# Syclus123/xDeepFM-pytorch

Measured on AMD Instinct MI355X. Metric: examples/sec (xDeepFM train step, Criteo-shape synthetic, bs=4096 per GPU), higher is better.
Workload: dtype f32

## Files before the change

include/xdfm.h:

```cpp
#ifndef XDFM_H
#define XDFM_H

#include <stddef.h>
#include <stdint.h>

#ifdef __cplusplus
extern "C" {
#endif

#define XDFM_ABI_VERSION 8

enum {
    XDFM_OK = 0,
    XDFM_ERR_INVALID = 1,
    XDFM_ERR_LAUNCH = 2,
    XDFM_ERR_NO_DEVICE = 3
};

enum { XDFM_ACT_LINEAR = 0, XDFM_ACT_RELU = 1, XDFM_ACT_SIGMOID = 2 };

int xdfm_abi_version(void);
const char* xdfm_last_error(void);
int xdfm_device_count(void);
int xdfm_set_option(const char* key, int value);
// ... 62 lines not shown
int xdfm_cin_fwd_pack(const float* W, int H, int Hp, int m, float* Wf, void* stream);
int xdfm_cin_level_fwd(const float* xp, const float* x0, const float* Wf, const float* bias,
                       int H, int Hp, int m, long N, int act, float* out, void* stream);

int xdfm_cin_level_fwd_ex_supported(int H, int Hp, int m, int D);
int xdfm_cin_level_fwd_ex(const float* xp, const float* x0, const float* Wf, const float* bias, int H, int Hp, int m, long N,
                          int act, float* out, int keep_rows, float* res, long ldres, int res_off, int dir0, int D,
                          unsigned* mask, long mask_ld, void* stream);

int xdfm_cin_direct_sum(const float* A, int row0, int rows, int B, int D,
                        float* res, long ldres, int off, void* stream);

int xdfm_cin_dout(const float* A, int H, int B, int D, int act,
                  const float* dHid, int hid0, int hid_rows,
                  const float* dDir, int dir_mode, long lddir, int dir_off, int dir0, int dir_rows,
                  float* dOut, float* dbias, void* stream);
size_t xdfm_cin_dout_ws_elems(int H, int B, int D);
int xdfm_cin_dout_det(const float* A, int H, int B, int D, int act,
                  const float* dHid, int hid0, int hid_rows,
                  const float* dDir, int dir_mode, long lddir, int dir_off, int dir0, int dir_rows,
                  float* dOut, float* dbias, float* ws, void* stream);

size_t xdfm_cin_bwd_pack_elems(int H, int Hp, int m);
int xdfm_cin_bwd_pack(const float* W, int H, int Hp, int m, float* Wz, void* stream);
int xdfm_cin_level_bwd_x(const float* dOut, const float* xp, const float* x0, const float* Wz,
                         int H, int Hp, int m, long N, float* dxp, float* dx0, void* stream);
enum { XDFM_BWX_SET_DXP = 1, XDFM_BWX_SET_DX0 = 2 };
int xdfm_cin_level_bwd_x_ex(const float* dOut, const float* xp, const float* x0, const float* Wz, int H, int Hp,
                            int m, long N, float* dxp, float* dx0, int flags, void* stream);

int xdfm_cin_bwd_x_is_folded(int H, int Hp, int m, int xp_is_x0);

size_t xdfm_cin_bwd_w_ws_elems(int H, int Hp, int m, long N);
int xdfm_cin_level_bwd_w(const float* dOut, const float* xp, const float* x0,
                         int H, int Hp, int m, long N, float* ws, float* dW, void* stream);

size_t xdfm_cin_bwd_prep_ws_elems(int H, int Hp, int m, int B, int D);
int xdfm_cin_bwd_nodout_supported(int H, int Hp, int m, int B, int D);
int xdfm_cin_level_bwd_x_src(const unsigned* mask, long mask_ld, const float* dHid, int hid_rows, const float* dDir, int dir_mode,
                             long lddir, int dir_off, int dir0, int dir_rows, int D, int h0, const float* xp, const float* x0,
                             const float* Wz, int H, int Hp, int m, long N, float* dxp, float* dx0, int flags, void* stream);
int xdfm_cin_bwd_prep(const float* A, const unsigned* mask, long mask_ld, int H, int B, int D, int act, const float* dHid,
                      int hid0, int hid_rows, const float* dDir, int dir_mode, long lddir, int dir_off, int dir0, int dir_rows,
                      float* dOut, float* dbias, float* dout_ws, const float* xp, const float* x0, int Hp, int m, float* bww_ws,
                      int* prepared, void* stream);
int xdfm_cin_level_bwd_w_prepared(const float* dOut, const float* xp, const float* x0, int H, int Hp, int m, long N,
                                  float* ws, float* dW, void* stream);

size_t xdfm_cin_attn_theta_elems(int D, int n_layers, int use_ln);
int xdfm_cin_attn_pool_fwd(const float* fm, int B, int S, int D, int nh, int n_layers, int use_ln, int use_res,
                           const float* theta, float* out, float* tok_save, float* o_save, float* ml_save,
                           float p_drop, const unsigned long long* drop_seed, void* stream);
int xdfm_cin_attn_pool_bwd(const float* fm, int B, int S, int D, int nh, int n_layers, int use_ln, int use_res,
                           const float* theta, const float* tok_save, const float* o_save, const float* ml_save,
                           const float* dout, float* dfm, float* dtheta, float p_drop,
                           const unsigned long long* drop_seed, void* stream);
size_t xdfm_cin_attn_pool_bwd_ws_elems(int B, int D, int n_layers, int use_ln);
int xdfm_cin_attn_pool_bwd_det(const float* fm, int B, int S, int D, int nh, int n_layers, int use_ln, int use_res,
                               const float* theta, const float* tok_save, const float* o_save, const float* ml_save,
                               const float* dout, float* dfm, float* dtheta, float* ws, float p_drop,
                               const unsigned long long* drop_seed, void* stream);
int xdfm_cin_attn_dropout_mask(int B, int S, int nh, int n_layers, float p_drop, const unsigned long long* drop_seed,
                               unsigned char* keep, void* stream);

int xdfm_l2_reg_fwd(const float* const* ptrs, const long* numel, const float* coeff, int T,
                    float* partials, float* out, void* stream);
int xdfm_l2_reg_bwd(const float* const* ptrs, const long* numel, const float* coeff, int T,
                    const float* gscale, float* gflat, const long* goff, int accumulate, void* stream);

typedef struct {
    const float* W;
    int H, Hp, m;
    float* fwd_pack;
    float* bwd_pack;
} xdfm_cin_pack_job;
int xdfm_cin_pack_all_supported(int H, int Hp, int m);
int xdfm_cin_pack_all(const xdfm_cin_pack_job* jobs, int L, void* stream);

size_t xdfm_colsum_ws_elems(int cols);
int xdfm_colsum(const float* g, long rows, int cols, long ld, float* ws, float* out, void* stream);
int xdfm_relu_bwd_colsum(const float* g, const float* y, long rows, int cols, long ldg, long ldy, float* ws, float* gz,
                         float* out, void* stream);

enum { XDFM_LINK_SIGMOID = 0, XDFM_LINK_IDENTITY = 1 };
enum { XDFM_LOSS_BCE = 0, XDFM_LOSS_MSE = 1, XDFM_LOSS_MAE = 2 };
size_t xdfm_head_ws_elems(int Ku, int Kv);
int xdfm_head_fwd(const float* lin, const float* u, const float* wu, int Ku, const float* v, const float* wv, int Kv,
                  const float* bias, const float* y, int B, float* pred, float* loss, float* ws, void* stream);
int xdfm_head_bwd(const float* pred, const float* y, const float* gloss, const float* u, const float* wu, int Ku,
                  const float* v, const float* wv, int Kv, int B, float* dlin, float* du, float* dv, float* grads,
                  float* ws, void* stream);
int xdfm_head_fwd_ex(const float* lin, const float* u, const float* wu, int Ku, const float* v, const float* wv, int Kv,
                     const float* bias, const float* y, int B, float* pred, float* loss_out, float* ws, int link, int loss,
                     void* stream);
int xdfm_head_bwd_ex(const float* pred, const float* y, const float* gloss, const float* u, const float* wu, int Ku,
                     const float* v, const float* wv, int Kv, int B, float* dlin, float* du, float* dv, float* grads,
                     float* ws, int link, int loss, void* stream);

typedef struct {
    float* param;
    float* grad;
    float* exp_avg;
    float* exp_avg_sq;
    const float* step;
    long numel;
    float l2;
    unsigned char* grad_marks;
    int flags;
    unsigned char* last;
} xdfm_adam_tensor;
enum { XDFM_ADAM_LAZY = 1, XDFM_ADAM_DEFERRED = 2 };
size_t xdfm_adam_step_ws_elems(int T);
int xdfm_adam_step(const xdfm_adam_tensor* tensors, int T, double lr, double beta1, double beta2, double eps,
                   float* l2_ws, float* l2_value, void* stream);
int xdfm_adam_step_lr(const xdfm_adam_tensor* tensors, int T, double lr, const double* lr_dev, double beta1, double beta2,
                      double eps, float* l2_ws, float* l2_value, void* stream);

typedef struct {
    float* param;
    float* grad;
    float* state;
    long numel;
    float l2;
    unsigned char* grad_marks;
} xdfm_opt_tensor;
size_t xdfm_opt_step_ws_elems(int T);
int xdfm_sgd_step(const xdfm_opt_tensor* tensors, int T, double lr, const double* lr_dev, float* l2_ws, float* l2_value,
                  void* stream);
int xdfm_adagrad_step(const xdfm_opt_tensor* tensors, int T, double lr, const double* lr_dev, double eps, float* l2_ws,
                      float* l2_value, void* stream);
int xdfm_rmsprop_step(const xdfm_opt_tensor* tensors, int T, double lr, const double* lr_dev, double alpha, double eps,
                      float* l2_ws, float* l2_value, void* stream);

typedef struct {
    int* clock;
    float* consts;
    int cap;
} xdfm_adam_clock;
int xdfm_adam_step_deferred(const xdfm_adam_tensor* tensors, int T, const xdfm_adam_clock* clk, double lr,
                            const double* lr_dev, double beta1, double beta2, double eps, float* l2_ws, float* l2_value,
                            void* stream);
typedef struct {
    float* const* param;
    float* const* exp_avg;
    float* const* exp_avg_sq;
    unsigned char* const* last;
    const float* l2;
    float* const* grad;
    unsigned char* const* marks;
} xdfm_adam_rows;
int xdfm_adam_catchup_rows(const float* X, long ldx, int B, const int* cols, const int* vocab, int m, int D,
                           const xdfm_adam_rows* emb, const xdfm_adam_rows* lin, const xdfm_adam_clock* clk,
                           double beta1, double beta2, double eps, float* backlog, void* stream);
int xdfm_adam_apply_rows(const float* X, long ldx, int B, const int* cols, const int* vocab, int m, int D,
                         const xdfm_adam_rows* emb, const xdfm_adam_rows* lin, const xdfm_adam_clock* clk,
                         double beta1, double beta2, double eps, float* l2_cell, float* l2_value, void* stream);
int xdfm_adam_flush(const xdfm_adam_tensor* tensors, int T, const xdfm_adam_clock* clk, double beta1, double beta2,
                    double eps, float* backlog, void* stream);

typedef struct {
    int* clock;
    float* rates;
    int cap;
    unsigned long long* backlog;
    unsigned long long* cell;
} xdfm_opt_clock;
// ... 79 lines not shown
```

xdeepfm-pytorch_amd/xdfm_amd/_lib.py:

```python
import ctypes
import os
from ctypes import c_char_p, c_double, c_float, c_int, c_long, c_size_t, c_void_p

import torch

_HERE = os.path.dirname(os.path.abspath(__file__))
LIB_PATH = os.environ.get("XDFM_LIB", os.path.join(_HERE, "libxdfm_hip.so"))

P = c_void_p
SIGNATURES = {
    "xdfm_abi_version": (c_int, []),
    "xdfm_last_error": (c_char_p, []),
    "xdfm_device_count": (c_int, []),
    "xdfm_set_option": (c_int, [c_char_p, c_int]),
    "xdfm_get_option": (c_int, [c_char_p]),
    "xdfm_graph_node_census": (c_int, [P, P, P, P]),
    "xdfm_set_ticket_board": (c_int, [P, c_int]),
    "xdfm_embed_gather_fwd": (c_int, [P, c_long, c_int, P, P, P, P, c_int, c_int, P, P, c_int, P, P, P, P, P]),
    "xdfm_embed_gather_fwd_ld": (c_int, [P, c_long, c_int, P, P, P, P, c_int, c_int, P, P, c_int, P, P, c_long, c_int, P, P, P]),
    "xdfm_varlen_pool_fwd": (c_int, [P, c_long, c_int, P, P, c_int, c_int, c_int, P, P, c_long, c_int, P, P, P, P]),
    "xdfm_varlen_pool_bwd_ws_elems": (c_size_t, [c_long, c_int, c_int, c_int]),
    "xdfm_varlen_pool_bwd": (c_int, [P, c_long, c_int, P, P, c_int, c_int, c_int, P, P, c_long, c_int, P, c_long, P, P, P, P, P, P,
                                     P, P]),
    "xdfm_varlen_pool_bwd_rows_ws_elems": (c_size_t, [c_long, c_int, c_int, c_int]),
# ... 7 lines not shown
    "xdfm_cin_pack_all": (c_int, [P, c_int, P]),
    "xdfm_cin_level_fwd": (c_int, [P, P, P, P, c_int, c_int, c_int, c_long, c_int, P, P]),
    "xdfm_cin_direct_sum": (c_int, [P, c_int, c_int, c_int, c_int, P, c_long, c_int, P]),
    "xdfm_cin_dout": (c_int, [P, c_int, c_int, c_int, c_int, P, c_int, c_int, P, c_int, c_long, c_int, c_int,
                              c_int, P, P, P]),
    "xdfm_cin_dout_ws_elems": (c_size_t, [c_int, c_int, c_int]),
    "xdfm_cin_dout_det": (c_int, [P, c_int, c_int, c_int, c_int, P, c_int, c_int, P, c_int, c_long, c_int, c_int,
                                  c_int, P, P, P, P]),
    "xdfm_cin_bwd_prep_ws_elems": (c_size_t, [c_int, c_int, c_int, c_int, c_int]),
    "xdfm_cin_bwd_prep": (c_int, [P, P, c_long, c_int, c_int, c_int, c_int, P, c_int, c_int, P, c_int, c_long, c_int, c_int, c_int, P, P, P,
                                  P, P, c_int, c_int, P, P, P]),
    "xdfm_cin_level_fwd_ex_supported": (c_int, [c_int, c_int, c_int, c_int]),
    "xdfm_cin_level_fwd_ex": (c_int, [P, P, P, P, c_int, c_int, c_int, c_long, c_int, P, c_int, P, c_long, c_int, c_int, c_int,
                                      P, c_long, P]),
    "xdfm_cin_bwd_nodout_supported": (c_int, [c_int, c_int, c_int, c_int, c_int]),
    "xdfm_cin_level_bwd_x_src": (c_int, [P, c_long, P, c_int, P, c_int, c_long, c_int, c_int, c_int, c_int, c_int, P, P, P, c_int, c_int,
                                         c_int, c_long, P, P, c_int, P]),
    "xdfm_cin_level_bwd_w_prepared": (c_int, [P, P, P, c_int, c_int, c_int, c_long, P, P, P]),
    "xdfm_cin_bwd_pack_elems": (c_size_t, [c_int, c_int, c_int]),
    "xdfm_cin_bwd_pack": (c_int, [P, c_int, c_int, c_int, P, P]),
    "xdfm_cin_level_bwd_x": (c_int, [P, P, P, P, c_int, c_int, c_int, c_long, P, P, P]),
    "xdfm_cin_level_bwd_x_ex": (c_int, [P, P, P, P, c_int, c_int, c_int, c_long, P, P, c_int, P]),
    "xdfm_cin_bwd_x_is_folded": (c_int, [c_int, c_int, c_int, c_int]),
    "xdfm_cin_bwd_w_ws_elems": (c_size_t, [c_int, c_int, c_int, c_long]),
    "xdfm_cin_level_bwd_w": (c_int, [P, P, P, c_int, c_int, c_int, c_long, P, P, P]),
    "xdfm_cin_attn_theta_elems": (c_size_t, [c_int, c_int, c_int]),
    "xdfm_cin_attn_pool_fwd": (c_int, [P, c_int, c_int, c_int, c_int, c_int, c_int, c_int, P, P, P, P, P, c_float, P, P]),
    "xdfm_cin_attn_pool_bwd": (c_int, [P, c_int, c_int, c_int, c_int, c_int, c_int, c_int, P, P, P, P, P, P, P, c_float,
                                       P, P]),
    "xdfm_cin_attn_pool_bwd_ws_elems": (c_size_t, [c_int, c_int, c_int, c_int]),
    "xdfm_cin_attn_pool_bwd_det": (c_int, [P, c_int, c_int, c_int, c_int, c_int, c_int, c_int, P, P, P, P, P, P, P, P, c_float,
                                           P, P]),
    "xdfm_cin_attn_dropout_mask": (c_int, [c_int, c_int, c_int, c_int, c_float, P, P, P]),
    "xdfm_head_ws_elems": (c_size_t, [c_int, c_int]),
    "xdfm_head_fwd": (c_int, [P, P, P, c_int, P, P, c_int, P, P, c_int, P, P, P, P]),
    "xdfm_head_bwd": (c_int, [P, P, P, P, P, c_int, P, P, c_int, c_int, P, P, P, P, P, P]),
    "xdfm_head_fwd_ex": (c_int, [P, P, P, c_int, P, P, c_int, P, P, c_int, P, P, P, c_int, c_int, P]),
    "xdfm_head_bwd_ex": (c_int, [P, P, P, P, P, c_int, P, P, c_int, c_int, P, P, P, P, P, c_int, c_int, P]),
    "xdfm_adam_step_ws_elems": (c_size_t, [c_int]),
    "xdfm_adam_step": (c_int, [P, c_int, c_double, c_double, c_double, c_double, P, P, P]),
    "xdfm_adam_step_lr": (c_int, [P, c_int, c_double, P, c_double, c_double, c_double, P, P, P]),
    "xdfm_adam_step_deferred": (c_int, [P, c_int, P, c_double, P, c_double, c_double, c_double, P, P, P]),
    "xdfm_adam_catchup_rows": (c_int, [P, c_long, c_int, P, P, c_int, c_int, P, P, P, c_double, c_double, c_double, P, P]),
    "xdfm_adam_apply_rows": (c_int, [P, c_long, c_int, P, P, c_int, c_int, P, P, P, c_double, c_double, c_double, P, P, P]),
    "xdfm_adam_flush": (c_int, [P, c_int, P, c_double, c_double, c_double, P, P]),
    "xdfm_adam_selftest": (c_int, [c_int, ctypes.c_ulonglong, ctypes.c_ulonglong, c_double, c_double, c_double, c_double, P, P]),
    "xdfm_opt_step_ws_elems": (c_size_t, [c_int]),
    "xdfm_sgd_step": (c_int, [P, c_int, c_double, P, P, P, P]),
    "xdfm_adagrad_step": (c_int, [P, c_int, c_double, P, c_double, P, P, P]),
    "xdfm_sgd_step_deferred": (c_int, [P, P, c_int, P, c_double, P, P, P, P]),
    "xdfm_adagrad_step_deferred": (c_int, [P, P, c_int, P, c_double, P, c_double, P, P, P]),
    "xdfm_opt_catchup_rows": (c_int, [c_int, P, c_long, c_int, P, P, c_int, c_int, P, P, P, c_double, P]),
    "xdfm_opt_flush": (c_int, [c_int, P, P, c_int, P, c_double, P]),
    "xdfm_rmsprop_step": (c_int, [P, c_int, c_double, P, c_double, c_double, P, P, P]),
    "xdfm_rmsprop_step_deferred": (c_int, [P, P, c_int, P, c_double, P, c_double, c_double, P, P, P]),
    "xdfm_rmsprop_catchup_rows": (c_int, [P, c_long, c_int, P, P, c_int, c_int, P, P, P, c_double, c_double, P]),
    "xdfm_rmsprop_flush": (c_int, [P, P, c_int, P, c_double, c_double, P]),
    "xdfm_vocab_lse_update": (c_int, [P, c_long, c_int, c_int, P, P, P]),
    "xdfm_vocab_softmax_grad": (c_int, [P, c_long, c_int, c_int, P, P, P]),
    "xdfm_vocab_ce_x3_supported": (c_int, [c_int]),
    "xdfm_vocab_ce_pack_elems": (c_long, [c_int, c_int]),
    "xdfm_vocab_ce_rows_padded": (c_long, [c_int]),
    "xdfm_vocab_ce_plan": (c_long, [c_int, P, c_int, c_int, P, P, c_long, P, P]),
    "xdfm_vocab_ce_pack_hidden": (c_int, [P, c_long, c_int, c_int, P, P]),
    "xdfm_vocab_ce_fwd": (c_int, [P, P, c_long, c_int, c_int, P, c_int, P, c_long, P, P, P, P, P, P]),
    "xdfm_vocab_ce_pack_g": (c_int, [P, c_int, c_int, P, P]),
    "xdfm_vocab_ce_bwd_h": (c_int, [P, c_int, c_int, P, c_int, P, c_long, P, P, P, P, P, P, P, c_long, P]),
    "xdfm_vocab_ce_bwd_w": (c_int, [P, c_int, c_int, P, c_int, c_int, P, P, P, P, P]),
    "xdfm_vocab_ce_pack_hidden_n": (c_int, [P, c_long, c_int, c_int, P, P, P]),
    "xdfm_vocab_ce_fwd_n": (c_int, [P, P, c_long, c_int, c_int, P, c_int, P, c_long, P, P, P, P, P, P, P]),
    "xdfm_vocab_ce_pack_g_n": (c_int, [P, c_int, c_int, P, P, P]),
    "xdfm_vocab_ce_bwd_h_n": (c_int, [P, c_int, c_int, P, c_int, P, c_long, P, P, P, P, P, P, P, c_long, P, P]),
    "xdfm_vocab_ce_bwd_w_n": (c_int, [P, c_int, c_int, P, c_int, c_int, P, P, P, P, P, P]),
    "xdfm_compact_rows_fwd": (c_int, [P, c_long, c_int, P, c_long, P, c_long, c_int, P, c_int, c_int, P, P, P, P, P, P, P, P]),
    "xdfm_compact_rows_bwd": (c_int, [P, c_long, P, c_long, c_int, P, P]),
    "xdfm_compact_rows_fwd_n": (c_int, [P, c_long, c_int, P, c_long, P, c_long, c_int, P, c_int, c_int, P, c_long, P, P, P, P, P, P, P, P]),
    "xdfm_autodis_supported": (c_int, [c_int, c_int]),
    "xdfm_autodis_ws_elems": (c_size_t, [c_long, c_int, c_int, c_int]),
    "xdfm_autodis_fwd": (c_int, [P, c_long, c_long, c_int, c_int, c_int, P, P, P, P, P]),
    "xdfm_autodis_bwd": (c_int, [P, c_long, c_long, c_int, c_int, c_int, P, P, P, P, c_long, c_int, P, P, P, P]),
    "xdfm_colsum_ws_elems": (c_size_t, [c_int]),
    "xdfm_colsum": (c_int, [P, c_long, c_int, c_long, P, P, P]),
    "xdfm_relu_bwd_colsum": (c_int, [P, P, c_long, c_int, c_long, c_long, P, P, P, P]),
    "xdfm_l2_reg_fwd": (c_int, [P, P, P, c_int, P, P, P]),
    "xdfm_l2_reg_bwd": (c_int, [P, P, P, c_int, P, P, P, c_int, P]),
}

class PackJob(ctypes.Structure):
    _fields_ = [("W", c_void_p), ("H", c_int), ("Hp", c_int), ("m", c_int), ("fwd_pack", c_void_p), ("bwd_pack", c_void_p)]


class VarLenField(ctypes.Structure):
    _fields_ = [("table", c_void_p), ("lin", c_void_p), ("col", c_int), ("maxlen", c_int), ("len_col", c_int), ("combiner", c_int),
                ("vocab", c_int), ("reserved", c_int)]


class AdamTensor(ctypes.Structure):
    _fields_ = [("param", c_void_p), ("grad", c_void_p), ("exp_avg", c_void_p), ("exp_avg_sq", c_void_p),
                ("step", c_void_p), ("numel", c_long), ("l2", ctypes.c_float), ("grad_marks", c_void_p), ("flags", c_int),
                ("last", c_void_p)]


class OptTensor(ctypes.Structure):
    _fields_ = [("param", c_void_p), ("grad", c_void_p), ("state", c_void_p), ("numel", c_long), ("l2", ctypes.c_float),
                ("grad_marks", c_void_p)]


class OptClock(ctypes.Structure):
    _fields_ = [("clock", c_void_p), ("rates", c_void_p), ("cap", c_int), ("backlog", c_void_p), ("cell", c_void_p)]


class OptRows(ctypes.Structure):
    _fields_ = [("param", c_void_p), ("state", c_void_p), ("last", c_void_p), ("l2", c_void_p)]


class AdamClock(ctypes.Structure):
    _fields_ = [("clock", c_void_p), ("consts", c_void_p), ("cap", c_int)]


class AdamRows(ctypes.Structure):
    _fields_ = [("param", c_void_p), ("exp_avg", c_void_p), ("exp_avg_sq", c_void_p), ("last", c_void_p), ("l2", c_void_p),
                ("grad", c_void_p), ("marks", c_void_p)]


ABI_VERSION = 8
_lib = None


class XdfmError(RuntimeError):
    pass


def load():
    global _lib
    if _lib is not None:
        return _lib
    if not os.path.exists(LIB_PATH):
        raise XdfmError(
            "libxdfm_hip.so not found at %s -- build it with `python __graft_entry__.py` "
            "(hipcc --offload-arch=gfx950); there is no CPU fallback for the xDeepFM hot path." % LIB_PATH)
    lib = ctypes.CDLL(LIB_PATH)
    for name, (res, args) in SIGNATURES.items():
        try:
            fn = getattr(lib, name)
        except AttributeError:
            raise XdfmError("libxdfm_hip.so at %s does not export %s (stale build?)" % (LIB_PATH, name))
        fn.restype = res
        fn.argtypes = args
    if lib.xdfm_abi_version() != ABI_VERSION:
        raise XdfmError("libxdfm_hip.so ABI %d != binding ABI %d" % (lib.xdfm_abi_version(), ABI_VERSION))
    _lib = lib
    return lib


def check(rc, what=""):
    if rc != 0:
        msg = load().xdfm_last_error().decode("utf-8", "replace")
        if rc == 1:
            raise ValueError("xdfm %s: %s" % (what, msg))
        raise XdfmError("xdfm %s failed (code %d): %s" % (what, rc, msg))


_BOARDS = {}


def ticket_board(device):
# ... 18 lines not shown
```

xdeepfm-pytorch_amd/xdfm_amd/ops.py:

```python
import ctypes
import os

import numpy as np
from typing import List, Optional, Sequence

import torch

from . import _lib

ACT_CODES = {"linear": 0, "relu": 1, "sigmoid": 2}

PROFILE = None


def _run(name, work, fn):
    if PROFILE is None:
        return fn()
    e0, e1 = torch.cuda.Event(enable_timing=True), torch.cuda.Event(enable_timing=True)
    e0.record()
    rc = fn()
    e1.record()
    PROFILE.append((name, work, e0, e1))
    return rc

# ... 654 lines not shown
    return CINStack.apply(x0_fm, B, D, tuple(layer_size), bool(split_half), act, pool, *params)


def to_fm_layout(x: torch.Tensor) -> torch.Tensor:
    B, R, D = x.shape
    return x.permute(1, 0, 2).reshape(R, B * D).contiguous()


def from_fm_layout(t: torch.Tensor, B: int, D: int) -> torch.Tensor:
    R = t.shape[0]
    return t.view(R, B, D).permute(1, 0, 2)


class AttnPool(torch.autograd.Function):

    @staticmethod
    def forward(ctx, fm, B, D, nh, n_layers, use_ln, use_res, p_drop, *params):
        _need_cuda(fm, "feature maps")
        lib = _lib.load()
        S = fm.shape[0]
        assert fm.shape[1] == B * D and fm.is_contiguous()
        theta = torch.cat([p.reshape(-1) for p in params])
        assert theta.numel() == lib.xdfm_cin_attn_theta_elems(D, n_layers, int(use_ln))
        dev = fm.device
        out = torch.empty((B, D), dtype=torch.float32, device=dev)
        tok = torch.empty((n_layers, B, S, D), dtype=torch.float32, device=dev)
        osv = torch.empty((n_layers, B, S, D), dtype=torch.float32, device=dev)
        ml = torch.empty((n_layers, B, S, nh, 2), dtype=torch.float32, device=dev)
        flops = 2.0 * 3 * D * S * S * B * n_layers
        p_drop = float(p_drop)
        seed = torch.randint(0, 2 ** 62, (1,), dtype=torch.int64, device=dev) if p_drop > 0 else None
        _lib.check(_run("cin_attn_pool_fwd", flops, lambda: lib.xdfm_cin_attn_pool_fwd(
            _ptr(fm), B, S, D, nh, n_layers, int(use_ln), int(use_res), _ptr(theta), _ptr(out), _ptr(tok), _ptr(osv),
            _ptr(ml), p_drop, _ptr(seed) if seed is not None else None, _stream())), "cin_attn_pool_fwd")
        ctx.cfg = (B, D, nh, n_layers, use_ln, use_res, p_drop, [tuple(p.shape) for p in params])
        ctx.drop_seed = seed
        AttnPool.last_drop_seed = seed
        ctx.save_for_backward(fm, theta, tok, osv, ml)
        return out

    @staticmethod
    def backward(ctx, dout):
        lib = _lib.load()
        fm, theta, tok, osv, ml = ctx.saved_tensors
        B, D, nh, n_layers, use_ln, use_res, p_drop, shapes = ctx.cfg
        seed = ctx.drop_seed
        S = fm.shape[0]
        dfm = torch.empty_like(fm)
        dtheta = torch.empty_like(theta)
        ws = torch.empty(lib.xdfm_cin_attn_pool_bwd_ws_elems(B, D, n_layers, int(use_ln)), dtype=torch.float32, device=fm.device)
        dout = dout.contiguous()
        flops = 2.0 * 7 * D * S * S * B * n_layers
        _lib.check(_run("cin_attn_pool_bwd", flops, lambda: lib.xdfm_cin_attn_pool_bwd_det(
            _ptr(fm), B, S, D, nh, n_layers, int(use_ln), int(use_res), _ptr(theta), _ptr(tok), _ptr(osv), _ptr(ml),
            _ptr(dout), _ptr(dfm), _ptr(dtheta), _ptr(ws), p_drop, _ptr(seed) if seed is not None else None, _stream())),
            "cin_attn_pool_bwd")
        grads, off = [], 0
        for sh in shapes:
            n = 1
            for k in sh:
                n *= k
            grads.append(dtheta[off:off + n].view(sh))
            off += n
        return (dfm, None, None, None, None, None, None, None) + tuple(grads)


def attn_pool(fm, B, D, mhsa_layers, layer_norms, pooling, use_res):
    params = []
    for l, att in enumerate(mhsa_layers):
        params += [att.W_q.weight, att.W_k.weight, att.W_v.weight, att.W_o.weight]
        if layer_norms is not None:
            params += [layer_norms[l].weight, layer_norms[l].bias]
    params += [pooling.attention[0].weight, pooling.attention[0].bias, pooling.attention[2].weight]
    nh = mhsa_layers[0].num_heads
    att0 = mhsa_layers[0]
    p_drop = float(att0.dropout.p) if att0.training else 0.0
    if any(float(a.dropout.p) != float(att0.dropout.p) for a in mhsa_layers):
        raise ValueError("cin_attn_pool: the attention layers must share one dropout rate")
    if p_drop >= 1.0:
        raise ValueError("cin_attn_pool: attention dropout must be < 1, got %g" % p_drop)
    return AttnPool.apply(fm, B, D, nh, len(mhsa_layers), layer_norms is not None, bool(use_res), p_drop, *params)


class Dense(torch.autograd.Function):

    @staticmethod
    def forward(ctx, x, W, b):
        ctx.save_for_backward(x, W)
        ctx.has_bias = b is not None
        return torch.nn.functional.linear(x, W, b)

    @staticmethod
    def backward(ctx, g):
        x, W = ctx.saved_tensors
        g = g.contiguous()
        dx = g.mm(W) if ctx.needs_input_grad[0] else None
        dW = g.t().mm(x) if ctx.needs_input_grad[1] else None
        db = None
        if ctx.has_bias and ctx.needs_input_grad[2]:
            lib = _lib.load()
            rows, cols = g.shape
            ws = torch.empty(lib.xdfm_colsum_ws_elems(cols), dtype=torch.float32, device=g.device)
            db = torch.empty(cols, dtype=torch.float32, device=g.device)
            _lib.check(lib.xdfm_colsum(_ptr(g), rows, cols, g.stride(0), _ptr(ws), _ptr(db), _stream()), "colsum")
        return dx, dW, db


class DenseReLU(torch.autograd.Function):

    @staticmethod
    def forward(ctx, x, W, b):
        y = torch._addmm_activation(b, x, W.t(), use_gelu=False)
        ctx.save_for_backward(x, W, y)
        return y

    @staticmethod
    def backward(ctx, g):
        x, W, y = ctx.saved_tensors
        lib = _lib.load()
        g = g.contiguous()
        rows, cols = g.shape
        ws = torch.empty(lib.xdfm_colsum_ws_elems(cols), dtype=torch.float32, device=g.device)
        gz = torch.empty_like(g)
        db = torch.empty(cols, dtype=torch.float32, device=g.device)
        _lib.check(lib.xdfm_relu_bwd_colsum(_ptr(g), _ptr(y), rows, cols, g.stride(0), y.stride(0), _ptr(ws), _ptr(gz),
                                            _ptr(db), _stream()), "relu_bwd_colsum")
        dx = gz.mm(W) if ctx.needs_input_grad[0] else None
        dW = gz.t().mm(x) if ctx.needs_input_grad[1] else None
        return dx, dW, db if ctx.needs_input_grad[2] else None


def dense_relu(x, W, b):
    if x.is_cuda and x.dim() == 2 and x.dtype == torch.float32 and b is not None and x.is_contiguous():
        return DenseReLU.apply(x, W, b)
    return torch.relu(dense(x, W, b))


def dense(x, W, b):
    if x.is_cuda and x.dim() == 2 and x.dtype == torch.float32:
        return Dense.apply(x, W, b)
    return torch.nn.functional.linear(x, W, b)


LINK_SIGMOID, LINK_IDENTITY = 0, 1
LOSS_BCE, LOSS_MSE, LOSS_MAE = 0, 1, 2


def head_mode(task, loss_func):
    link = {"binary": LINK_SIGMOID, "regression": LINK_IDENTITY}.get(task) if isinstance(task, str) else None
    if link is None or isinstance(loss_func, (list, tuple)):
        return None
    F = torch.nn.functional
    for fn, loss in ((F.binary_cross_entropy, LOSS_BCE), (F.mse_loss, LOSS_MSE), (F.l1_loss, LOSS_MAE)):
        if loss_func is fn:
            return None if (link == LINK_IDENTITY and loss == LOSS_BCE) else (link, loss)
    return None


class Head(torch.autograd.Function):

    @staticmethod
    def forward(ctx, y, bias, lin, u, wu, v, wv, link=LINK_SIGMOID, loss=LOSS_BCE):
        lib = _lib.load()
        yv = y.reshape(-1).contiguous()
        B = yv.numel()
        dev = yv.device
        linv = lin.reshape(-1).contiguous() if lin is not None else None
        u = u.contiguous() if u is not None else None
        v = v.contiguous() if v is not None else None
        wu = wu.reshape(-1).contiguous() if wu is not None else None
        wv = wv.reshape(-1).contiguous() if wv is not None else None
        Ku = u.shape[1] if u is not None else 0
        Kv = v.shape[1] if v is not None else 0
        for t, k in ((u, Ku), (v, Kv)):
            if t is not None and (t.dim() != 2 or t.shape[0] != B):
                raise ValueError("xdfm head: operands must be [B, K]")
        pred = torch.empty(B, dtype=torch.float32, device=dev)
        out = torch.empty(1, dtype=torch.float32, device=dev)
        ws = torch.empty(lib.xdfm_head_ws_elems(Ku, Kv), dtype=torch.float32, device=dev)
        _lib.check(lib.xdfm_head_fwd_ex(_ptr(linv), _ptr(u), _ptr(wu), Ku, _ptr(v), _ptr(wv), Kv, _ptr(bias), _ptr(yv), B,
                                        _ptr(pred), _ptr(out), _ptr(ws), int(link), int(loss), _stream()), "head_fwd")
        ctx.save_for_backward(pred, yv, u, wu, v, wv)
        ctx.cfg = (bias is not None, lin is not None, tuple(lin.shape) if lin is not None else None, Ku, Kv)
        ctx.mode = (int(link), int(loss))
        ctx.mark_non_differentiable(pred)
        ctx.set_materialize_grads(False)
        return pred, out

    @staticmethod
    def backward(ctx, _gpred, gloss):
        if gloss is None:
            return (None,) * 9
        lib = _lib.load()
        pred, yv, u, wu, v, wv = ctx.saved_tensors
        has_bias, has_lin, lin_shape, Ku, Kv = ctx.cfg
        B = pred.numel()
        dev = pred.device
        f32 = dict(dtype=torch.float32, device=dev)
        dlin = torch.empty(B, **f32) if has_lin else None
        du = torch.empty((B, Ku), **f32) if u is not None else None
        dv = torch.empty((B, Kv), **f32) if v is not None else None
# ... 449 lines not shown
```

Before: 2.030 million.

## Add native MFMA dense backward kernels fusing ReLU mask and bias grad

Adds a custom MFMA fp32 GEMM kernel for dense layers. Backward now computes dx with the ReLU mask applied on the fly, and computes dW with a split-K reduction that also produces the bias gradient, replacing the separate relu_bwd_colsum kernel plus two rocBLAS GEMMs. The forward native path exists but is disabled by default. It removes the intermediate gz buffer and some launches, at the risk that a hand-written kernel is slower than rocBLAS for the MLP shapes.

```diff
diff --git a/include/xdfm.h b/include/xdfm.h
--- a/include/xdfm.h
+++ b/include/xdfm.h
@@ -168,6 +168,15 @@
 int xdfm_relu_bwd_colsum(const float* g, const float* y, long rows, int cols, long ldg, long ldy, float* ws, float* gz,
                          float* out, void* stream);
 
+int xdfm_dense_supported(long rows, int in, int out);
+size_t xdfm_dense_bwd_w_ws_elems(long rows, int in, int out);
+int xdfm_dense_fwd(const float* x, long rows, int in, long ldx, const float* W, int out, const float* b, int act, float* y,
+                   long ldy, void* stream);
+int xdfm_dense_bwd_x(const float* g, long ldg, const float* y, long ldy, long rows, int out, const float* W, int in, float* dx,
+                     long lddx, void* stream);
+int xdfm_dense_bwd_w(const float* g, long ldg, const float* y, long ldy, const float* x, long ldx, long rows, int in, int out,
+                     float* ws, float* dW, float* db, void* stream);
+
 enum { XDFM_LINK_SIGMOID = 0, XDFM_LINK_IDENTITY = 1 };
 enum { XDFM_LOSS_BCE = 0, XDFM_LOSS_MSE = 1, XDFM_LOSS_MAE = 2 };
 size_t xdfm_head_ws_elems(int Ku, int Kv);
diff --git a/xdeepfm-pytorch_amd/csrc/dnn.hip b/xdeepfm-pytorch_amd/csrc/dnn.hip
--- /dev/null
+++ b/xdeepfm-pytorch_amd/csrc/dnn.hip
@@ -0,0 +1,300 @@
+#include "xdfm_internal.h"
+
+#define DN_T 64
+#define DN_K 32
+#define DN_NW 8
+#define DN_E 4
+#define DN_PLANE (DN_T * 4 + 8)
+#define DN_TILE (8 * DN_PLANE)
+#define DN_SPLIT_ROWS 256
+#define DN_MAX_SPLIT 32
+#define DN_MAX_DIM (1 << 20)
+
+struct DnArgs {
+    const float* A; const float* Ay; long lda, lday;
+    const float* B; long ldb;
+    float* C; long ldc, cslab;
+    const float* bias; int relu;
+    float* dbpart;
+    long M, N, K, kper;
+};
+
+__device__ __forceinline__ int dn_lds(int p, int m) { return p * DN_PLANE + (m << 2); }
+
+template <bool KC, bool MASK>
+struct DnStage {
+    float v[DN_E], y[DN_E];
+    long off[DN_E], offy[DN_E];
+    unsigned fixed, ok;
+    __device__ __forceinline__ void init(long ld, long ldy, long m0, long mdim) {
+        const int t = threadIdx.x;
+        fixed = 0;
+        if (KC) {
+#pragma unroll
+            for (int e = 0; e < DN_E; ++e) {
+                const long m = m0 + (t >> 5) + 2 * DN_NW * e;
+                if (m < mdim) fixed |= 1u << e;
+                const long mc = m < mdim ? m : mdim - 1;
+                off[e] = mc * ld;
+                offy[e] = mc * ldy;
+            }
+        } else {
+            const long m = m0 + (t & 63);
+            if (m < mdim) fixed = (1u << DN_E) - 1;
+            off[0] = offy[0] = m < mdim ? m : mdim - 1;
+        }
+    }
+    __device__ __forceinline__ void load(const float* __restrict__ src, const float* __restrict__ ysrc, long ld, long ldy,
+                                         long k0, long kend) {
+        const int t = threadIdx.x;
+        if (KC) {
+            const long k = k0 + (t & 31);
+            const long kc = k < kend ? k : kend - 1;
+            ok = k < kend ? fixed : 0u;
+#pragma unroll
+            for (int e = 0; e < DN_E; ++e) {
+                v[e] = src[off[e] + kc];
+                if (MASK) y[e] = ysrc[offy[e] + kc];
+            }
+        } else {
+            const int q = t >> 6;
+            const long kb = k0 + 8 * (q >> 1) + (q & 1);
+            if (k0 + DN_K <= kend) {
+                ok = fixed;
+                const float* pv = src + kb * ld + off[0];
+                const float* py = MASK ? ysrc + kb * ldy + off[0] : nullptr;
+#pragma unroll
+                for (int e = 0; e < DN_E; ++e) {
+                    v[e] = pv[2 * e * ld];
+                    if (MASK) y[e] = py[2 * e * ldy];
+                }
+            } else {
+                ok = 0;
+#pragma unroll
+                for (int e = 0; e < DN_E; ++e) {
+                    const long k = kb + 2 * e;
+                    const long kc = k < kend ? k : kend - 1;
+                    if (k < kend) ok |= 1u << e;
+                    v[e] = src[kc * ld + off[0]];
+                    if (MASK) y[e] = ysrc[kc * ldy + off[0]];
+                }
+                ok &= fixed;
+            }
+        }
+    }
+    __device__ __forceinline__ float store(float* __restrict__ tile) {
+        const int t = threadIdx.x;
+#pragma unroll
+        for (int e = 0; e < DN_E; ++e) {
+            const bool live = (ok >> e & 1u) && (!MASK || y[e] > 0.f);
+            v[e] = live ? v[e] : 0.f;
+        }
+        if (KC) {
+            const int k = t & 31, p = (k >> 3) * 2 + (k & 1);
+#pragma unroll
+            for (int e = 0; e < DN_E; ++e) tile[dn_lds(p, (t >> 5) + 2 * DN_NW * e) + ((k >> 1) & 3)] = v[e];
+        } else {
+            f32x4 q = {v[0], v[1], v[2], v[3]};
+            *(f32x4*)(tile + dn_lds(t >> 6, t & 63)) = q;
+        }
+        float s = 0.f;
+#pragma unroll
+        for (int e = 0; e < DN_E; ++e) s += v[e];
+        return s;
+    }
+};
+
+enum { DN_EPI_FWD = 0, DN_EPI_PLAIN = 1, DN_EPI_SLAB = 2 };
+
+template <bool AKC, bool BKC, bool MASK, int EPI>
+__global__ __launch_bounds__(DN_NW * 64) void dense_mfma_kernel(DnArgs a) {
+    __shared__ __attribute__((aligned(16))) float lds[4 * DN_TILE];
+    const int t = threadIdx.x, lane = t & 63, w = t >> 6, c = lane & 31, s = lane >> 5;
+    const int wt = w & 3, kh = w >> 2;
+    const int wm = (wt & 1) * 32, wn = (wt >> 1) * 32;
+    const long m0 = (long)blockIdx.x * DN_T, n0 = (long)blockIdx.y * DN_T;
+    const long kbeg = (long)blockIdx.z * a.kper;
+    const long kend = kbeg + a.kper < a.K ? kbeg + a.kper : a.K;
+    const int steps = (int)((kend - kbeg + DN_K - 1) / DN_K);
+
+    DnStage<AKC, MASK> sa;
+    DnStage<BKC, false> sb;
+    sa.init(a.lda, a.lday, m0, a.M);
+    sb.init(a.ldb, 0, n0, a.N);
+    f32x16 acc;
+#pragma unroll
+    for (int r = 0; r < 16; ++r) acc[r] = 0.f;
+    float bsum = 0.f;
+
+    sa.load(a.A, a.Ay, a.lda, a.lday, kbeg, kend);
+    sb.load(a.B, nullptr, a.ldb, 0, kbeg, kend);
+    bsum += sa.store(lds);
+    sb.store(lds + DN_TILE);
+    __syncthreads();
+    for (int it = 0; it < steps; ++it) {
+        const float* As = lds + (it & 1) * 2 * DN_TILE;
+        const float* Bs = As + DN_TILE;
+        const bool more = it + 1 < steps;
+        if (more) {
+            const long k0 = kbeg + (long)(it + 1) * DN_K;
+            sa.load(a.A, a.Ay, a.lda, a.lday, k0, kend);
+            sb.load(a.B, nullptr, a.ldb, 0, k0, kend);
+        }
+#pragma unroll
+        for (int u = 0; u < 2; ++u) {
+            const int p = (2 * kh + u) * 2 + s;
+            const f32x4 af = *(const f32x4*)(As + dn_lds(p, wm + c));
+            const f32x4 bf = *(const f32x4*)(Bs + dn_lds(p, wn + c));
+#pragma unroll
+            for (int j = 0; j < 4; ++j) acc = __builtin_amdgcn_mfma_f32_32x32x2f32(af[j], bf[j], acc, 0, 0, 0);
+        }
+        if (more) {
+            float* nxt = lds + ((it + 1) & 1) * 2 * DN_TILE;
+            bsum += sa.store(nxt);
+            sb.store(nxt + DN_TILE);
+        }
+        __syncthreads();
+    }
+    if (kh == 1) {
+#pragma unroll
+        for (int r = 0; r < 16; ++r) lds[(wt * 16 + r) * 64 + lane] = acc[r];
+    }
+    __syncthreads();
+    if (kh == 0) {
+#pragma unroll
+        for (int r = 0; r < 16; ++r) acc[r] += lds[(wt * 16 + r) * 64 + lane];
+        float* C = a.C + (long)blockIdx.z * a.cslab;
+        const long col = n0 + wn + c;
+        float bv = 0.f;
+        if (EPI == DN_EPI_FWD && a.bias && col < a.N) bv = a.bias[col];
+#pragma unroll
+        for (int r = 0; r < 16; ++r) {
+            const long row = m0 + wm + frag_row(r, s);
+            if (row >= a.M || col >= a.N) continue;
+            float v = acc[r];
+            if (EPI == DN_EPI_FWD) {
+                v += bv;
+                if (a.relu) v = v < 0.f ? 0.f : v;
+            }
+            C[row * a.ldc + col] = v;
+        }
+    }
+    if (EPI == DN_EPI_SLAB) {
+        if (a.dbpart && blockIdx.y == 0) {
+            __syncthreads();
+            lds[t] = bsum;
+            __syncthreads();
+            if (t < DN_T && m0 + t < a.M)
+                a.dbpart[(long)blockIdx.z * a.M + m0 + t] = ((lds[t] + lds[64 + t]) + (lds[128 + t] + lds[192 + t])) +
+                                                            ((lds[256 + t] + lds[320 + t]) + (lds[384 + t] + lds[448 + t]));
+        }
+    }
+}
+
+__global__ __launch_bounds__(256) void dense_bwd_w_finish_kernel(const float* __restrict__ ws, int nsplit, long mn, long m,
+                                                                 float* __restrict__ dW, float* __restrict__ db) {
+    const long e = (long)blockIdx.x * 256 + threadIdx.x;
+    const long total = mn + (db ? m : 0);
+    if (e >= total) return;
+    const float* p = e < mn ? ws + e : ws + (long)nsplit * mn + (e - mn);
+    const long pitch = e < mn ? mn : m;
+    float sum = 0.f;
+    int z = 0;
+    for (; z + 4 <= nsplit; z += 4) {
+        const float v0 = p[(long)z * pitch], v1 = p[(long)(z + 1) * pitch], v2 = p[(long)(z + 2) * pitch], v3 = p[(long)(z + 3) * pitch];
+        sum = (((sum + v0) + v1) + v2) + v3;
+    }
+    for (; z < nsplit; ++z) sum += p[(long)z * pitch];
+    if (e < mn) dW[e] = sum;
+    else db[e - mn] = sum;
+}
+
+static inline bool dn_supported(long rows, long in, long out) {
+    return rows >= 1 && rows < (1L << 31) && in >= 1 && in <= DN_MAX_DIM && out >= 32 && out <= DN_MAX_DIM && out % 32 == 0;
+}
+static inline int dn_splits(long rows) {
+    const long n = (rows + DN_SPLIT_ROWS - 1) / DN_SPLIT_ROWS;
+    return (int)(n < 1 ? 1 : (n > DN_MAX_SPLIT ? DN_MAX_SPLIT : n));
+}
+
+#define DN_LAUNCH(AKC, BKC, MASK, EPI, grid, st, a) \
+    hipLaunchKernelGGL((dense_mfma_kernel<AKC, BKC, MASK, EPI>), grid, dim3(DN_NW * 64), 0, st, a)
+
+extern "C" {
+
+int xdfm_dense_supported(long rows, int in, int out) { return dn_supported(rows, in, out) ? 1 : 0; }
+
+size_t xdfm_dense_bwd_w_ws_elems(long rows, int in, int out) {
+    if (!dn_supported(rows, in, out)) return 0;
+    return (size_t)dn_splits(rows) * ((size_t)out * in + out);
+}
+
+int xdfm_dense_fwd(const float* x, long rows, int in, long ldx, const float* W, int out, const float* b, int act, float* y,
+                   long ldy, void* stream) {
+    XDFM_REQUIRE(x && W && y, "dense_fwd: null pointer");
+    XDFM_REQUIRE(rows > 0, "dense_fwd: rows = %ld", rows);
+    XDFM_REQUIRE(in > 0, "dense_fwd: in = %d", in);
+    XDFM_REQUIRE(dn_supported(rows, in, out), "dense_fwd: unsupported shape rows = %ld, in = %d, out = %d (out must be a multiple of 32)",
+                 rows, in, out);
+    XDFM_REQUIRE(ldx >= in, "dense_fwd: ldx = %ld < in = %d", ldx, in);
+    XDFM_REQUIRE(ldy >= out, "dense_fwd: ldy = %ld < out = %d", ldy, out);
+    XDFM_REQUIRE(act == XDFM_ACT_LINEAR || act == XDFM_ACT_RELU, "dense_fwd: act = %d (0 = none, 1 = relu)", act);
+    DnArgs a{};
+    a.A = x; a.lda = ldx; a.B = W; a.ldb = in; a.C = y; a.ldc = ldy; a.bias = b; a.relu = act == XDFM_ACT_RELU;
+    a.M = rows; a.N = out; a.K = in; a.kper = round_up(in, DN_K);
+    const dim3 grid(ceil_div(rows, DN_T), ceil_div(out, DN_T), 1);
+    DN_LAUNCH(true, true, false, DN_EPI_FWD, grid, (hipStream_t)stream, a);
+    return xdfm_check_launch("dense_fwd");
+}
+
+int xdfm_dense_bwd_x(const float* g, long ldg, const float* y, long ldy, long rows, int out, const float* W, int in, float* dx,
+                     long lddx, void* stream) {
+    XDFM_REQUIRE(g && W && dx, "dense_bwd_x: null pointer");
+    XDFM_REQUIRE(rows > 0, "dense_bwd_x: rows = %ld", rows);
+    XDFM_REQUIRE(in > 0, "dense_bwd_x: in = %d", in);
+    XDFM_REQUIRE(dn_supported(rows, in, out), "dense_bwd_x: unsupported shape rows = %ld, in = %d, out = %d (out must be a multiple of 32)",
+                 rows, in, out);
+    XDFM_REQUIRE(ldg >= out, "dense_bwd_x: ldg = %ld < out = %d", ldg, out);
+    XDFM_REQUIRE(!y || ldy >= out, "dense_bwd_x: ldy = %ld < out = %d", ldy, out);
+    XDFM_REQUIRE(lddx >= in, "dense_bwd_x: lddx = %ld < in = %d", lddx, in);
+    DnArgs a{};
+    a.A = g; a.Ay = y; a.lda = ldg; a.lday = ldy; a.B = W; a.ldb = in; a.C = dx; a.ldc = lddx;
+    a.M = rows; a.N = in; a.K = out; a.kper = round_up(out, DN_K);
+    const dim3 grid(ceil_div(rows, DN_T), ceil_div(in, DN_T), 1);
+    if (y) DN_LAUNCH(true, false, true, DN_EPI_PLAIN, grid, (hipStream_t)stream, a);
+    else DN_LAUNCH(true, false, false, DN_EPI_PLAIN, grid, (hipStream_t)stream, a);
+    return xdfm_check_launch("dense_bwd_x");
+}
+
+int xdfm_dense_bwd_w(const float* g, long ldg, const float* y, long ldy, const float* x, long ldx, long rows, int in, int out,
+                     float* ws, float* dW, float* db, void* stream) {
+    XDFM_REQUIRE(g && x && dW, "dense_bwd_w: null pointer");
+    XDFM_REQUIRE(rows > 0, "dense_bwd_w: rows = %ld", rows);
+    XDFM_REQUIRE(in > 0, "dense_bwd_w: in = %d", in);
+    XDFM_REQUIRE(dn_supported(rows, in, out), "dense_bwd_w: unsupported shape rows = %ld, in = %d, out = %d (out must be a multiple of 32)",
+                 rows, in, out);
+    XDFM_REQUIRE(ws, "dense_bwd_w: workspace is NULL (xdfm_dense_bwd_w_ws_elems floats)");
+    XDFM_REQUIRE(ldg >= out, "dense_bwd_w: ldg = %ld < out = %d", ldg, out);
+    XDFM_REQUIRE(!y || ldy >= out, "dense_bwd_w: ldy = %ld < out = %d", ldy, out);
+    XDFM_REQUIRE(ldx >= in, "dense_bwd_w: ldx = %ld < in = %d", ldx, in);
+    hipStream_t st = (hipStream_t)stream;
+    const int want = dn_splits(rows);
+    const long kper = round_up(ceil_div(rows, want), DN_K);
+    const int nsplit = ceil_div(rows, kper);
+    const long mn = (long)out * in;
+    DnArgs a{};
+    a.A = g; a.Ay = y; a.lda = ldg; a.lday = ldy; a.B = x; a.ldb = ldx;
+    a.M = out; a.N = in; a.K = rows; a.kper = kper; a.ldc = in;
+    if (nsplit == 1) { a.C = dW; a.cslab = 0; a.dbpart = db; }
+    else { a.C = ws; a.cslab = mn; a.dbpart = db ? ws + (long)nsplit * mn : nullptr; }
+    const dim3 grid(ceil_div(out, DN_T), ceil_div(in, DN_T), nsplit);
+    if (y) DN_LAUNCH(false, false, true, DN_EPI_SLAB, grid, st, a);
+    else DN_LAUNCH(false, false, false, DN_EPI_SLAB, grid, st, a);
+    if (nsplit > 1) {
+        const long total = mn + (db ? out : 0);
+        hipLaunchKernelGGL(dense_bwd_w_finish_kernel, dim3(ceil_div(total, 256)), dim3(256), 0, st, ws, nsplit, mn, (long)out, dW, db);
+    }
+    return xdfm_check_launch("dense_bwd_w");
+}
+
+}
diff --git a/xdeepfm-pytorch_amd/xdfm_amd/_lib.py b/xdeepfm-pytorch_amd/xdfm_amd/_lib.py
--- a/xdeepfm-pytorch_amd/xdfm_amd/_lib.py
+++ b/xdeepfm-pytorch_amd/xdfm_amd/_lib.py
@@ -113,6 +113,11 @@
     "xdfm_colsum_ws_elems": (c_size_t, [c_int]),
     "xdfm_colsum": (c_int, [P, c_long, c_int, c_long, P, P, P]),
     "xdfm_relu_bwd_colsum": (c_int, [P, P, c_long, c_int, c_long, c_long, P, P, P, P]),
+    "xdfm_dense_supported": (c_int, [c_long, c_int, c_int]),
+    "xdfm_dense_bwd_w_ws_elems": (c_size_t, [c_long, c_int, c_int]),
+    "xdfm_dense_fwd": (c_int, [P, c_long, c_int, c_long, P, c_int, P, c_int, P, c_long, P]),
+    "xdfm_dense_bwd_x": (c_int, [P, c_long, P, c_long, c_long, c_int, P, c_int, P, c_long, P]),
+    "xdfm_dense_bwd_w": (c_int, [P, c_long, P, c_long, P, c_long, c_long, c_int, c_int, P, P, P, P]),
     "xdfm_l2_reg_fwd": (c_int, [P, P, P, c_int, P, P, P]),
     "xdfm_l2_reg_bwd": (c_int, [P, P, P, c_int, P, P, P, c_int, P]),
 }
diff --git a/xdeepfm-pytorch_amd/xdfm_amd/ops.py b/xdeepfm-pytorch_amd/xdfm_amd/ops.py
--- a/xdeepfm-pytorch_amd/xdfm_amd/ops.py
+++ b/xdeepfm-pytorch_amd/xdfm_amd/ops.py
@@ -760,17 +760,79 @@
     return AttnPool.apply(fm, B, D, nh, len(mhsa_layers), layer_norms is not None, bool(use_res), p_drop, *params)
 
 
+def _env_switch(environ, key, default=True):
+    v = environ.get(key)
+    return default if v is None else v != "0"
+
+
+DNN_NATIVE = _env_switch(os.environ, "XDFM_DNN_NATIVE")
+DNN_NATIVE_FWD = False
+
+
+def _ld(t):
+    return max(int(t.stride(0)), int(t.shape[1]))
+
+
+def _rows_ok(t):
+    return t.stride(1) == 1 and (t.shape[0] == 1 or t.stride(0) >= t.shape[1])
+
+
+def dense_native(x, W, b=None):
+    if not (DNN_NATIVE and x.is_cuda and W.is_cuda and x.dim() == 2 and W.dim() == 2 and x.dtype == torch.float32
+            and W.dtype == torch.float32 and x.shape[0] >= 1 and x.shape[1] == W.shape[1] and W.is_contiguous() and _rows_ok(x)):
+        return False
+    if b is not None and not (b.is_cuda and b.dtype == torch.float32 and b.dim() == 1 and b.is_contiguous()):
+        return False
+    return bool(_lib.load().xdfm_dense_supported(x.shape[0], x.shape[1], W.shape[0]))
+
+
+def _dense_fwd_native(x, W, b, act):
+    lib = _lib.load()
+    rows, k = x.shape
+    out = W.shape[0]
+    y = torch.empty(rows, out, dtype=torch.float32, device=x.device)
+    _lib.check(_run("dense_fwd", 0.0, lambda: lib.xdfm_dense_fwd(_ptr(x), rows, k, _ld(x), _ptr(W), out, _ptr(b), act, _ptr(y), out,
+                                                                 _stream())), "dense_fwd")
+    return y
+
+
+def _dense_bwd_native(g, y, x, W, need_dx, need_dw, need_db):
+    lib = _lib.load()
+    rows, k = x.shape
+    out = W.shape[0]
+    if not _rows_ok(g):
+        g = g.contiguous()
+    ldy = _ld(y) if y is not None else 0
+    dx = dW = db = None
+    if need_dx:
+        dx = torch.empty(rows, k, dtype=torch.float32, device=g.device)
+        _lib.check(_run("dense_bwd_x", 0.0, lambda: lib.xdfm_dense_bwd_x(_ptr(g), _ld(g), _ptr(y), ldy, rows, out, _ptr(W), k, _ptr(dx), k,
+                                                                         _stream())), "dense_bwd_x")
+    if need_dw or need_db:
+        ws = torch.empty(lib.xdfm_dense_bwd_w_ws_elems(rows, k, out), dtype=torch.float32, device=g.device)
+        dW = torch.empty(out, k, dtype=torch.float32, device=g.device)
+        db = torch.empty(out, dtype=torch.float32, device=g.device) if need_db else None
+        _lib.check(_run("dense_bwd_w", 0.0, lambda: lib.xdfm_dense_bwd_w(_ptr(g), _ld(g), _ptr(y), ldy, _ptr(x), _ld(x), rows, k, out,
+                                                                         _ptr(ws), _ptr(dW), _ptr(db), _stream())), "dense_bwd_w")
+    return dx, dW if need_dw else None, db
+
+
 class Dense(torch.autograd.Function):
 
     @staticmethod
     def forward(ctx, x, W, b):
         ctx.save_for_backward(x, W)
         ctx.has_bias = b is not None
+        if DNN_NATIVE_FWD and dense_native(x, W, b):
+            return _dense_fwd_native(x, W, b, ACT_CODES["linear"])
         return torch.nn.functional.linear(x, W, b)
 
     @staticmethod
     def backward(ctx, g):
         x, W = ctx.saved_tensors
+        if dense_native(x, W):
+            return _dense_bwd_native(g, None, x, W, ctx.needs_input_grad[0], ctx.needs_input_grad[1],
+                                     ctx.has_bias and ctx.needs_input_grad[2])
         g = g.contiguous()
         dx = g.mm(W) if ctx.needs_input_grad[0] else None
         dW = g.t().mm(x) if ctx.needs_input_grad[1] else None
@@ -788,13 +850,18 @@
 
     @staticmethod
     def forward(ctx, x, W, b):
-        y = torch._addmm_activation(b, x, W.t(), use_gelu=False)
+        if DNN_NATIVE_FWD and dense_native(x, W, b):
+            y = _dense_fwd_native(x, W, b, ACT_CODES["relu"])
+        else:
+            y = torch._addmm_activation(b, x, W.t(), use_gelu=False)
         ctx.save_for_backward(x, W, y)
         return y
 
     @staticmethod
     def backward(ctx, g):
         x, W, y = ctx.saved_tensors
+        if dense_native(x, W):
+            return _dense_bwd_native(g, y, x, W, *ctx.needs_input_grad)
         lib = _lib.load()
         g = g.contiguous()
         rows, cols = g.shape
```

New measurement: 2.056 million (median of 6 runs). 1.2% higher.
